# kdavila/lecturemath

Measured on AMD Instinct MI355X. Metric: frames/sec end-to-end binarize+CC+group @1080p, higher is better.
Workload: dtype u8

## Files before the change

lecturemath_amd/csrc/lm_api.hip:

```cpp
#include "lm_common.h"
#include "lm_stream.h"

#include <stdarg.h>
#include <stdlib.h>
#include <stdio.h>
#include <string.h>

#include "../../include/lecturemath_amd.h"

#include "lm_cc_kernels.hip"
#include "lm_fcn_bytes.hip"
#include "lm_match_kernels.hip"
#include "lm_match_batch.hip"
#include "lm_group.hip"
#include "lm_fcn.hip"
#include "lm_fcn2.hip"

static thread_local char g_err[512] = "";

void lm_set_error(const char* fmt, ...)
{
    va_list ap;
    va_start(ap, fmt);
    vsnprintf(g_err, sizeof(g_err), fmt, ap);
// ... 333 lines not shown
        return LM_ERR_ARG;
    }
    const LmGeom g = c->g;
    hipStream_t st = (hipStream_t)stream;
    if ((long long)g.H * ((g.W + 3) / 4) >= (1ll << 24) && d_labels) { lm_set_error("lm_label_batch: frame too large for the label writer (H*W/4 must be < 2^24)"); return LM_ERR_ARG; }
#if !LM_HIP_EMULATED
    {
        LM_HIP(hipFuncSetAttribute((const void*)lm_k_band, hipFuncAttributeMaxDynamicSharedMemorySize, (int)lm_band_smem(c)));
    }
#endif
    if (lm_profile_mark(c, st, true, n_frames)) return LM_ERR_HIP;
    static const int want_parts = [] { const char* e = getenv("LM_LABEL_PARTS"); const int v = e ? atoi(e) : LM_LABEL_PARTS; return (v >= 1 && v <= 8) ? v : LM_LABEL_PARTS; }();
    int parts = want_parts;
    while (parts > 1 && n_frames / parts < LM_LABEL_PART_MIN) parts--;
    if (parts > 1 && !c->aux_stream) {
        LM_HIP(hipStreamCreateWithFlags((hipStream_t*)&c->aux_stream, hipStreamNonBlocking));
        LM_HIP(hipEventCreateWithFlags((hipEvent_t*)&c->ev_fork, hipEventDisableTiming));
        LM_HIP(hipEventCreateWithFlags((hipEvent_t*)&c->ev_join, hipEventDisableTiming));
    }
    if (parts <= 1) {
        const int rc = lm_label_launch(c, src, 0, n_frames, d_labels, st);
        if (rc) return rc;
    } else {
        hipStream_t aux = (hipStream_t)c->aux_stream;
        LM_HIP(hipEventRecord((hipEvent_t)c->ev_fork, st));
        LM_HIP(hipStreamWaitEvent(aux, (hipEvent_t)c->ev_fork, 0));
        int rc = LM_OK;
        for (int k = 0, f0 = 0; k < parts && rc == LM_OK; k++) {
            const int n = n_frames / parts + (k < n_frames % parts ? 1 : 0);
            rc = lm_label_launch(c, src, f0, n, d_labels, (k & 1) ? aux : st);
            f0 += n;
        }
        const hipError_t e1 = hipEventRecord((hipEvent_t)c->ev_join, aux);
        const hipError_t e2 = (e1 == hipSuccess) ? hipStreamWaitEvent(st, (hipEvent_t)c->ev_join, 0) : e1;
        if (e2 != hipSuccess) {
            (void)hipStreamSynchronize(aux);
            if (rc == LM_OK) { lm_set_error("lm_label_batch: joining the second queue failed: %s", hipGetErrorString(e2)); rc = LM_ERR_HIP; }
        }
        if (rc) return rc;
    }
    if (lm_profile_mark(c, st, false, n_frames)) return LM_ERR_HIP;
    c->last_batch = n_frames;
    c->last_fused = src.logits ? 1 : 0;
    c->stats_fresh = 1;
    return LM_OK;
}

extern "C" int lm_label_batch(LmCtx* c, const uint8_t* d_binary, int n_frames, int32_t* d_labels, void* stream)
{
    LmLabelSrc src = {d_binary, nullptr, 0.0f, 0u, nullptr};
    return lm_label_batch_src(c, src, n_frames, d_labels, stream);
}

extern "C" int lm_label_batch_logits(LmCtx* c, const float* d_logits, int n_frames, int thr, int invert, uint8_t* d_binary, int32_t* d_labels, void* stream)
{
    if (!c || !d_logits || n_frames <= 0 || n_frames > c->max_batch) {
        lm_set_error("lm_label_batch_logits: bad arguments (n_frames=%d, max_batch=%d)", n_frames, c ? c->max_batch : -1);
        return LM_ERR_ARG;
    }
    const LmGeom g = c->g;
    float edge = 0.0f;
    int cmp = 0;
    const bool shape_ok = (g.W & 3) == 0 && ((((uintptr_t)d_logits) & 15) == 0) && (!d_binary || ((((uintptr_t)d_binary) & 3) == 0));
    {
        const int rc = lm_threshold_form(shape_ok && !getenv("LM_LABEL_UNFUSED"), thr, (hipStream_t)stream, &edge, &cmp);
        if (rc) return rc;
    }
    if (cmp) {
        LmLabelSrc src = {nullptr, d_logits, edge, invert ? 0xffu : 0u, d_binary};
        return lm_label_batch_src(c, src, n_frames, d_labels, stream);
    }
    if (!d_binary) { lm_set_error("lm_label_batch_logits: this frame shape / threshold needs the two-pass path, which needs d_binary"); return LM_ERR_ARG; }
    const int rc = lm_threshold(d_logits, d_binary, (int64_t)n_frames * g.W * g.H, thr, invert, stream);
    if (rc) return rc;
    return lm_label_batch(c, d_binary, n_frames, d_labels, stream);
}

extern "C" int lm_label_was_fused(LmCtx* c) { return c ? c->last_fused : 0; }

extern "C" int lm_label_counts(LmCtx* c, int32_t* h_counts, void* stream)
{
    if (!c || !h_counts || c->last_batch <= 0) { lm_set_error("lm_label_counts: no labelled batch"); return LM_ERR_STATE; }
    LM_HIP(hipMemcpyAsync(h_counts, c->n_labels, (size_t)c->last_batch * sizeof(int32_t), hipMemcpyDeviceToHost,
                          (hipStream_t)stream));
    LM_HIP(hipStreamSynchronize((hipStream_t)stream));
    if (g_band_stamps && getenv("LM_DEBUG_BAND_STAMPS")) {
        const size_t n = (size_t)c->nbands * c->last_batch * 8;
        unsigned long long* h = (unsigned long long*)malloc(n * sizeof(unsigned long long));
        if (h && hipMemcpy(h, g_band_stamps, n * sizeof(unsigned long long), hipMemcpyDeviceToHost) == hipSuccess) {
            FILE* f = fopen(getenv("LM_DEBUG_BAND_STAMPS"), "wb");
            if (f) { fwrite(h, sizeof(unsigned long long), n, f); fclose(f); }
        }
        free(h);
    }
    return LM_OK;
}

extern "C" int lm_cc_stats_batch(LmCtx* c, void* stream)
{
    if (!c || c->last_batch <= 0) { lm_set_error("lm_cc_stats_batch: no labelled batch"); return LM_ERR_STATE; }
    const LmGeom g = c->g;
    hipStream_t st = (hipStream_t)stream;
    const int B = c->last_batch;
    if (!c->stats_fresh)
        hipLaunchKernelGGL(lm_k_stats_init, dim3(32, B), dim3(256), 0, st, c->st_min_y, c->st_max_y, c->st_min_x, c->st_max_x,
                           c->st_count, c->n_labels, g.W, g.H, g.cap);
    c->stats_fresh = 0;
    hipLaunchKernelGGL(lm_k_stats, dim3((g.WW + LM_ST_WORDS - 1) / LM_ST_WORDS, (g.H + LM_ST_ROWS - 1) / LM_ST_ROWS, B), dim3(256), 0,
                       st, c->bits, c->starts, c->prefix, c->rowoff, c->final_label, c->st_min_y, c->st_max_y, c->st_min_x,
                       c->st_max_x, c->st_count, g.WW, g.H, g.cap);
    LM_HIP(hipGetLastError());
    return LM_OK;
}

extern "C" int lm_cc_stats_read(LmCtx* c, int frame, int n, int32_t* h_mins_y, int32_t* h_maxs_y, int32_t* h_mins_x,
                                int32_t* h_maxs_x, int32_t* h_counts, void* stream)
{
    if (!c || frame < 0 || frame >= c->last_batch || n < 0 || n > c->g.cap) {
        lm_set_error("lm_cc_stats_read: bad arguments");
        return LM_ERR_ARG;
    }
    hipStream_t st = (hipStream_t)stream;
    const size_t off = (size_t)frame * c->g.cap, nb = (size_t)n * sizeof(int32_t);
    if (n > 0) {
        if (h_mins_y) LM_HIP(hipMemcpyAsync(h_mins_y, c->st_min_y + off, nb, hipMemcpyDeviceToHost, st));
        if (h_maxs_y) LM_HIP(hipMemcpyAsync(h_maxs_y, c->st_max_y + off, nb, hipMemcpyDeviceToHost, st));
        if (h_mins_x) LM_HIP(hipMemcpyAsync(h_mins_x, c->st_min_x + off, nb, hipMemcpyDeviceToHost, st));
        if (h_maxs_x) LM_HIP(hipMemcpyAsync(h_maxs_x, c->st_max_x + off, nb, hipMemcpyDeviceToHost, st));
// ... 48 lines not shown
                                int* out_maxs_y, int* out_mins_x, int* out_maxs_x, int* out_counts, float* output_age)
{
    if (count_labels <= 0 || width <= 0 || height <= 0) return 0;
    LmCtx* c = lm_host_ctx(width, height);
    const size_t px = (size_t)width * height;
    if (!c || lm_stage(c, px)) return 0;
    const int n = count_labels;
    int32_t* d_out = nullptr;
    if (hipMalloc((void**)&d_out, (size_t)n * 9 * sizeof(int32_t)) != hipSuccess) { lm_set_error("CC_AgeBoundaries: hipMalloc failed"); return 0; }
    int32_t *mny = d_out, *mxy = d_out + n, *mnx = d_out + 2 * (size_t)n, *mxx = d_out + 3 * (size_t)n, *cnt = d_out + 4 * (size_t)n,
            *ageb = d_out + 5 * (size_t)n, *last_px = d_out + 7 * (size_t)n, *last_neg = d_out + 8 * (size_t)n;
    float* agef = (float*)(d_out + 6 * (size_t)n);
    bool ok = hipMemcpy(c->stage_i32, labels, px * sizeof(int32_t), hipMemcpyHostToDevice) == hipSuccess;
    if (ok && ages) ok = hipMemcpy(c->stage_f32, ages, px * sizeof(float), hipMemcpyHostToDevice) == hipSuccess;
    if (ok) {
        const float* d_ages = ages ? c->stage_f32 : (const float*)nullptr;
        hipLaunchKernelGGL(lm_k_ab_init, dim3(lm_blocks(n, 256)), dim3(256), 0, (hipStream_t)0, mny, mxy, mnx, mxx, cnt, ageb, last_px, last_neg,
                           width, height, n);
        hipLaunchKernelGGL(lm_k_ab_scan, dim3(lm_blocks((long long)px, 256)), dim3(256), 0, (hipStream_t)0, c->stage_i32, d_ages, width, height, n,
                           mny, mxy, mnx, mxx, cnt, last_px, last_neg);
        hipLaunchKernelGGL(lm_k_ab_age, dim3(lm_blocks((long long)px, 256)), dim3(256), 0, (hipStream_t)0, c->stage_i32, d_ages, width, height, n,
                           last_neg, ageb);
        hipLaunchKernelGGL(lm_k_ab_finish, dim3(lm_blocks(n, 256)), dim3(256), 0, (hipStream_t)0, ageb, last_px, last_neg, d_ages, agef, n);
        const size_t nb = (size_t)n * sizeof(int32_t);
        ok = hipMemcpy(out_mins_y, mny, nb, hipMemcpyDeviceToHost) == hipSuccess &&
             hipMemcpy(out_maxs_y, mxy, nb, hipMemcpyDeviceToHost) == hipSuccess &&
             hipMemcpy(out_mins_x, mnx, nb, hipMemcpyDeviceToHost) == hipSuccess &&
             hipMemcpy(out_maxs_x, mxx, nb, hipMemcpyDeviceToHost) == hipSuccess &&
             hipMemcpy(out_counts, cnt, nb, hipMemcpyDeviceToHost) == hipSuccess &&
             hipMemcpy(output_age, agef, nb, hipMemcpyDeviceToHost) == hipSuccess;
    }
    if (!ok) lm_set_error("CC_AgeBoundaries: device copy/launch failed");
    (void)hipFree(d_out);
    return 0;
}

extern "C" void lm_stream_destroy(LmStream* s)
{
    if (!s) return;
    void* ptrs[] = {s->cc, s->assign, s->frame_cc_off, s->crop, s->chash, s->active_cc, s->active_box, s->active_last, s->active, s->counters, s->best,
                    s->batch_cc_base, s->batch_word_base};
    for (void* p : ptrs)
        if (p) (void)hipFree(p);
    if (s->mb) {
        LmMatchBatch* m = s->mb;
        void* mp[] = {m->nt_cnt, m->nt_src, m->tlast, m->tcur[0], m->tcur[1], m->ftile_all, m->nt_foff, m->nt_list, m->cls, m->troot, m->rootpos, m->ftile, m->s_prefix, m->tcount[0], m->tcount[1], m->toff[0], m->toff[1], m->pairs[0], m->pairs[1], m->pair_u[0],
                      m->pair_u[1], m->sidx, m->s_list, m->s_box, m->newpos, m->n_src, m->ttab, m->tkey, m->twin, m->big[0], m->big[1], m->n_big};
        for (void* p : mp)
            if (p) (void)hipFree(p);
        delete m;
    }
    for (int i = 0; i < s->n_run_events; i++) (void)hipEventDestroy(s->run_events[i]);
    free(s->run_events);
    if (s->rd_scratch) (void)hipFree(s->rd_scratch);
    if (s->garena) (void)hipFree(s->garena);
    if (s->gpin) (void)hipHostFree(s->gpin);
    delete s;
}

extern "C" int lm_stream_set_min_pixels(LmStream* s, int min_pixels)
{
    if (!s || min_pixels < 0) { lm_set_error("lm_stream_set_min_pixels: bad arguments"); return LM_ERR_ARG; }
    s->min_pixels = min_pixels;
    return LM_OK;
}

extern "C" int lm_stream_reset(LmStream* s, void* stream)
{
    if (!s) { lm_set_error("lm_stream_reset: null stream"); return LM_ERR_ARG; }
    LM_HIP(hipMemsetAsync(s->counters, 0, sizeof(LmCounters), (hipStream_t)stream));
    LM_HIP(hipMemsetAsync(s->best, 0xff, (size_t)s->ctx->g.cap * sizeof(unsigned long long), (hipStream_t)stream));
    LM_HIP(hipMemsetAsync(s->frame_cc_off, 0, sizeof(long long), (hipStream_t)stream));
    LM_HIP(hipMemsetAsync(s->chash, 0, (size_t)s->cap_cc * sizeof(uint32_t), (hipStream_t)stream));
    if (s->mb) LM_HIP(hipMemsetAsync(s->mb->ttab, 0xff, (size_t)LM_MB_TTAB * sizeof(unsigned long long), (hipStream_t)stream));
    s->frames_pushed = 0;
    s->frames_matched = 0;
    s->tempo_B = 0;
    return LM_OK;
}

extern "C" LmStream* lm_stream_create(LmCtx* ctx, int max_frames, int64_t max_ccs, int64_t max_crop_words, int max_uniques,
                                      double min_recall, double min_precision, int max_gap, int min_pixels)
{
    if (!ctx || max_frames <= 0 || max_ccs <= 0 || max_crop_words <= 0 || max_uniques <= 0) {
        lm_set_error("lm_stream_create: bad arguments");
        return nullptr;
    }
    LmStream* s = new LmStream();
    memset(s, 0, sizeof(*s));
    s->ctx = ctx;
    s->cap_frames = max_frames;
    s->cap_cc = max_ccs;
    s->cap_words = (unsigned long long)max_crop_words;
    s->cap_uniq = max_uniques;
    s->min_recall = min_recall;
    s->min_precision = min_precision;
    s->max_gap = max_gap;
    s->min_pixels = min_pixels;
    int rc = LM_OK;
    rc |= lm_alloc(&s->cc, (size_t)max_ccs);
    rc |= lm_alloc(&s->assign, (size_t)max_ccs);
    rc |= lm_alloc(&s->frame_cc_off, (size_t)max_frames + 1);
    rc |= lm_alloc(&s->crop, (size_t)max_crop_words);
    rc |= lm_alloc(&s->chash, (size_t)max_ccs);
    rc |= lm_alloc(&s->active_cc, (size_t)max_uniques);
    rc |= lm_alloc(&s->active_box, (size_t)max_uniques);
    rc |= lm_alloc(&s->active_last, (size_t)max_uniques);
    rc |= lm_alloc(&s->active, (size_t)max_uniques);
    rc |= lm_alloc(&s->best, (size_t)ctx->g.cap);
    rc |= lm_alloc(&s->counters, (size_t)1);
    rc |= lm_alloc(&s->batch_cc_base, (size_t)ctx->max_batch);
    rc |= lm_alloc(&s->batch_word_base, (size_t)ctx->max_batch);
    {
        LmMatchBatch* m = new LmMatchBatch();
        memset(m, 0, sizeof(*m));
        s->mb = m;
        m->cap_tiles = (int)(max_ccs / LM_MB_TILE) + max_frames + 2;
        long long cp = 16 * (long long)max_ccs;
        if (cp < (1 << 16)) cp = 1 << 16;
        if (cp > (1 << 23)) cp = 1 << 23;
        m->cap_pairs = (uint32_t)cp;
        rc |= lm_alloc(&m->ftile, (size_t)max_frames + 2);
        rc |= lm_alloc(&m->s_prefix, (size_t)max_frames + 2);
        rc |= lm_alloc(&m->ftile_all, (size_t)max_frames + 2);
        rc |= lm_alloc(&m->nt_foff, (size_t)max_frames + 2);
        rc |= lm_alloc(&m->nt_list, (size_t)max_ccs);
        rc |= lm_alloc(&m->cls, (size_t)max_ccs);
        rc |= lm_alloc(&m->troot, (size_t)max_ccs);
        rc |= lm_alloc(&m->rootpos, (size_t)max_ccs);
        rc |= lm_alloc(&m->nt_cnt, (size_t)LM_MB_MAX_FRAMES);
        rc |= lm_alloc(&m->nt_src, (size_t)max_ccs);
        rc |= lm_alloc(&m->tlast, (size_t)max_ccs);
        for (int k = 0; k < 2; k++) {
            rc |= lm_alloc(&m->tcount[k], (size_t)m->cap_tiles + 1);
            rc |= lm_alloc(&m->toff[k], (size_t)m->cap_tiles + 1);
            rc |= lm_alloc(&m->tcur[k], ((size_t)m->cap_tiles + 1) * LM_MB_JY);
            rc |= lm_alloc(&m->pairs[k], (size_t)m->cap_pairs);
            rc |= lm_alloc(&m->pair_u[k], (size_t)m->cap_pairs);
        }
        rc |= lm_alloc(&m->sidx, (size_t)max_ccs);
        rc |= lm_alloc(&m->s_list, (size_t)max_ccs);
        rc |= lm_alloc(&m->s_box, (size_t)max_ccs);
        rc |= lm_alloc(&m->newpos, (size_t)max_ccs);
        rc |= lm_alloc(&m->n_src, (size_t)1);
        rc |= lm_alloc(&m->ttab, (size_t)LM_MB_TTAB);
        rc |= lm_alloc(&m->tkey, (size_t)max_ccs);
        rc |= lm_alloc(&m->twin, (size_t)max_ccs);
        m->cap_big = 1u << 16;
        rc |= lm_alloc(&m->big[0], (size_t)m->cap_big);
        rc |= lm_alloc(&m->big[1], (size_t)m->cap_big);
        rc |= lm_alloc(&m->n_big, (size_t)2);
#if !LM_HIP_EMULATED
        if (rc == LM_OK &&
            hipFuncSetAttribute((const void*)lm_k_mb_resolve, hipFuncAttributeMaxDynamicSharedMemorySize, (int)LM_MB_RESOLVE_SMEM) != hipSuccess)
            rc = LM_ERR_HIP;
#endif
        const char* e = getenv("LM_MATCH_PER_FRAME");
        s->match_per_frame = (e && atoi(e) == 1) ? 1 : 0;
    }
    if (rc == LM_OK && hipMemset(s->mb->twin, 0, (size_t)max_ccs) != hipSuccess) rc = LM_ERR_HIP;
    if (rc == LM_OK) rc = lm_stream_reset(s, nullptr);
    if (rc == LM_OK && hipStreamSynchronize(nullptr) != hipSuccess) rc = LM_ERR_HIP;
    if (rc != LM_OK) {
        lm_stream_destroy(s);
        return nullptr;
    }
    return s;
}

static void lm_launch_match(LmStream* s, int f, hipStream_t st)
{
    hipLaunchKernelGGL(lm_k_match, LM_HIP_EMULATED ? dim3(2, 2) : dim3(16, 64), dim3(256), 0, st, s->cc, s->crop, s->frame_cc_off, f,
                       s->active_box, s->active_last, s->active_cc, s->counters, s->best, s->min_recall, s->min_precision, s->max_gap);
    hipLaunchKernelGGL(lm_k_update, dim3(1), dim3(1024), 0, st, s->cc, s->frame_cc_off, f, s->active, s->active_cc, s->active_box,
                       s->active_last, s->counters, s->assign, s->best, s->max_gap, s->cap_uniq, (f & 15) == 15 ? 1 : 0);
}

static void lm_flush_tempo(LmStream* s, hipStream_t st)
{
    if (s->tempo_B <= 0) return;
    const LmMatchBatch mb = *s->mb;
    hipLaunchKernelGGL(lm_k_mb_tempo, dim3(LM_HIP_EMULATED ? 2 : 1024), dim3(256), 0, st, s->cc, s->frame_cc_off, s->tempo_f0, s->tempo_B, s->active_box,
                       s->active_cc, s->active_last, s->counters, mb, s->max_gap, s->active, s->assign);
    s->tempo_B = 0;
}

static void lm_launch_match_frames(LmStream* s, int f0, int n, hipStream_t st, hipEvent_t ev_pre = nullptr, bool defer_tempo = false)
{
    if (!s->match_per_frame) lm_flush_tempo(s, st);
    if (s->match_per_frame) {
        for (int i = 0; i < n; i++) lm_launch_match(s, f0 + i, st);
        return;
    }
    const LmMatchBatch mb = *s->mb;
    const dim3 gj(LM_HIP_EMULATED ? 2 : 128, LM_HIP_EMULATED ? 2 : LM_MB_JY), gt(LM_HIP_EMULATED ? 2 : 1024), ge(LM_HIP_EMULATED ? 2 : 2048), gb(LM_HIP_EMULATED ? 2 : 1024);
    for (int done = 0; done < n;) {
        const int B = (n - done < LM_MB_MAX_FRAMES) ? n - done : LM_MB_MAX_FRAMES;
        const int f = f0 + done;
        s->last_match_frames = B;
        const int twins = (s->min_recall <= 1.0 && s->min_precision <= 1.0) ? 1 : 0;
        if (twins) {
            const dim3 gc(LM_HIP_EMULATED ? 2 : 256);
            hipLaunchKernelGGL(lm_k_mb_twin_insert, gc, dim3(256), 0, st, s->cc, s->chash, s->frame_cc_off, f, B, s->counters, mb);
            hipLaunchKernelGGL(lm_k_mb_twin_probe, gc, dim3(256), 0, st, s->cc, s->frame_cc_off, f, B, s->counters, mb, s->max_gap);
            hipLaunchKernelGGL(lm_k_mb_twin_cmp, ge, dim3(256), 0, st, s->cc, s->crop, s->frame_cc_off, f, B, s->counters, mb);
            hipLaunchKernelGGL(lm_k_mb_twin_final, gc, dim3(256), 0, st, s->cc, s->frame_cc_off, f, B, s->counters, mb);
        }
        hipLaunchKernelGGL(lm_k_mb_nt, dim3(B + 1), dim3(1024), 0, st, s->frame_cc_off, f, B, s->active, s->active_cc, s->active_box, s->active_last,
                           s->counters, mb, s->max_gap, twins);
        hipLaunchKernelGGL((lm_k_mb_join<0, 0>), gj, dim3(256), 0, st, s->cc, s->frame_cc_off, f, B, s->active_box, s->active_cc, s->counters, mb);
        hipLaunchKernelGGL((lm_k_mb_join<0, 1>), gj, dim3(256), 0, st, s->cc, s->frame_cc_off, f, B, s->active_box, s->active_cc, s->counters, mb);
        hipLaunchKernelGGL((lm_k_mb_eval<0>), ge, dim3(256), 0, st, s->cc, s->crop, s->frame_cc_off, f, B, s->active_last, s->counters, mb,
                           s->min_recall, s->min_precision, s->max_gap);
        hipLaunchKernelGGL((lm_k_mb_eval_big<0>), gb, dim3(256), 0, st, s->cc, s->crop, s->active_last, s->counters, mb, s->min_recall, s->min_precision,
                           s->max_gap);
        hipLaunchKernelGGL(lm_k_mb_sources, dim3(1), dim3(1024), 0, st, s->cc, s->frame_cc_off, f, B, s->counters, mb);
        hipLaunchKernelGGL((lm_k_mb_join<1, 0>), gj, dim3(256), 0, st, s->cc, s->frame_cc_off, f, B, s->active_box, s->active_cc, s->counters, mb);
        hipLaunchKernelGGL((lm_k_mb_join<1, 1>), gj, dim3(256), 0, st, s->cc, s->frame_cc_off, f, B, s->active_box, s->active_cc, s->counters, mb);
        hipLaunchKernelGGL((lm_k_mb_eval<1>), ge, dim3(256), 0, st, s->cc, s->crop, s->frame_cc_off, f, B, s->active_last, s->counters, mb,
                           s->min_recall, s->min_precision, s->max_gap);
        hipLaunchKernelGGL((lm_k_mb_eval_big<1>), gb, dim3(256), 0, st, s->cc, s->crop, s->active_last, s->counters, mb, s->min_recall, s->min_precision,
                           s->max_gap);
        if (ev_pre && done + B >= n) (void)hipEventRecord(ev_pre, st);
        hipLaunchKernelGGL(lm_k_mb_resolve, dim3(1), dim3(LM_MB_RT), LM_MB_RESOLVE_SMEM, st, s->cc, s->frame_cc_off, f, B, s->active, s->active_cc,
                           s->active_box, s->active_last, s->counters, s->assign, mb, s->max_gap, s->cap_uniq);
        if (defer_tempo && done + B >= n) { s->tempo_f0 = f; s->tempo_B = B; }
        else
            hipLaunchKernelGGL(lm_k_mb_tempo, gt, dim3(256), 0, st, s->cc, s->frame_cc_off, f, B, s->active_box, s->active_cc, s->active_last,
                               s->counters, mb, s->max_gap, s->active, s->assign);
        done += B;
    }
}

static int lm_stream_emit_batch(LmStream* s, int B, void* stream)
{
    LmCtx* c = s->ctx;
    const LmGeom g = c->g;
    hipStream_t st = (hipStream_t)stream;
    int rc = lm_cc_stats_batch(c, stream);
    if (rc) return rc;
    hipLaunchKernelGGL(lm_k_select, dim3(B), dim3(1024), 0, st, c->st_min_y, c->st_max_y, c->st_min_x, c->st_max_x,
                       c->st_count, c->n_labels, c->kept_label, c->kept_cropoff, c->frame_kept, c->frame_cropwords, g.cap,
                       s->min_pixels);
    hipLaunchKernelGGL(lm_k_batch_offsets, dim3(1), dim3(1024), 0, st, c->frame_kept, c->frame_cropwords, B, s->counters,
                       s->frame_cc_off, s->batch_cc_base, s->batch_word_base, s->cap_cc, s->cap_words, s->cap_frames);
    hipLaunchKernelGGL(lm_k_emit, dim3(LM_HIP_EMULATED ? 2 : LM_EMIT_GRID, B), dim3(256), 0, st, c->bits, c->starts, c->prefix, c->rowoff, c->final_label,
                       c->st_min_y, c->st_max_y, c->st_min_x, c->st_max_x, c->st_count, c->kept_label, c->kept_cropoff,
                       c->frame_kept, c->frame_cropwords, s->batch_cc_base, s->batch_word_base, s->cc, s->crop, s->chash, s->frames_pushed, g.WW,
                       g.H, g.cap);
    LM_HIP(hipGetLastError());
    return LM_OK;
}

extern "C" int lm_stream_push_labelled(LmStream* s, int n_frames, void* stream)
{
    if (!s || n_frames <= 0 || n_frames != s->ctx->last_batch) {
        lm_set_error("lm_stream_push_labelled: %d frames, the context's last labelled batch has %d", n_frames, s ? s->ctx->last_batch : 0);
        return LM_ERR_ARG;
    }
    if (s->frames_pushed + n_frames > s->cap_frames) {
// ... 31 lines not shown
            lm_launch_match_frames(s, s->frames_pushed, B, st);
            s->frames_matched += B;
        }
        LM_HIP(hipGetLastError());
        s->frames_pushed += B;
        done += B;
    }
    return LM_OK;
}

extern "C" int lm_stream_push(LmStream* s, const uint8_t* d_binary, int n_frames, int32_t* d_labels, void* stream)
{
    return lm_stream_push_impl(s, d_binary, n_frames, d_labels, 1, stream);
}

extern "C" int lm_stream_push_records(LmStream* s, const uint8_t* d_binary, int n_frames, int32_t* d_labels, void* stream)
{
    return lm_stream_push_impl(s, d_binary, n_frames, d_labels, 0, stream);
}

static int lm_run_events(LmStream* s, int want)
{
    if (want <= s->n_run_events) return LM_OK;
    want += 192;
    hipEvent_t* ev = (hipEvent_t*)realloc(s->run_events, (size_t)want * sizeof(hipEvent_t));
    if (!ev) { lm_set_error("lm_stream_run_logits: out of memory"); return LM_ERR_HIP; }
    s->run_events = ev;
    for (; s->n_run_events < want; s->n_run_events++) LM_HIP(hipEventCreateWithFlags(&s->run_events[s->n_run_events], hipEventDisableTiming));
    return LM_OK;
}

extern "C" int lm_stream_run_logits(LmStream* s, const float* d_logits, int n_frames, int batch, uint8_t* d_binary, int32_t* d_labels, int thr,
                                    int do_match, int schedule, void* stream_wide, void* stream_match)
{
    if (!s || !d_logits || n_frames < 0 || batch <= 0 || batch > s->ctx->max_batch || schedule < 0 || schedule > 1) {
        lm_set_error("lm_stream_run_logits: bad arguments (batch %d, context batch %d, schedule %d)", batch, s ? s->ctx->max_batch : 0, schedule);
        return LM_ERR_ARG;
    }
    if (do_match && s->frames_matched != s->frames_pushed) {
        lm_set_error("lm_stream_run_logits: %d frames pushed without matching; call lm_stream_match first", s->frames_pushed - s->frames_matched);
        return LM_ERR_STATE;
    }
    hipStream_t sw = (hipStream_t)stream_wide, sm = (hipStream_t)stream_match;
    const bool two = do_match && sm != sw;
    const bool gated = two && schedule == 1 && batch <= LM_MB_MAX_FRAMES && !s->match_per_frame;
    const size_t px = (size_t)s->ctx->g.W * s->ctx->g.H;
    const int nb = (n_frames + batch - 1) / batch;
    if (two) { const int rc = lm_run_events(s, 3 * nb); if (rc) return rc; }
    hipEvent_t* ev = s->run_events;
    int prev_n = 0;
    for (int k = 0, f0 = 0; f0 < n_frames; f0 += batch, k++) {
        const int n = (n_frames - f0 < batch) ? n_frames - f0 : batch;
        if (gated && k >= 2) LM_HIP(hipStreamWaitEvent(sw, ev[3 * (k - 2) + 2], 0));
        int rc = lm_label_batch_logits(s->ctx, d_logits + (size_t)f0 * px, n, thr, 1, d_binary, d_labels, stream_wide);
        if (rc) return rc;
        if (gated) LM_HIP(hipEventRecord(ev[3 * k], sw));
        rc = lm_stream_push_labelled(s, n, stream_wide);
        if (rc) return rc;
        if (!do_match) continue;
        if (!two) {
            rc = lm_stream_match(s, n, stream_wide);
            if (rc) return rc;
        } else if (!gated) {
            LM_HIP(hipEventRecord(ev[3 * k + 1], sw));
            LM_HIP(hipStreamWaitEvent(sm, ev[3 * k + 1], 0));
            rc = lm_stream_match(s, n, stream_match);
            if (rc) return rc;
        } else {
            LM_HIP(hipEventRecord(ev[3 * k + 1], sw));
            if (k >= 1) {
                LM_HIP(hipStreamWaitEvent(sm, ev[3 * k], 0));
                lm_launch_match_frames(s, s->frames_matched, prev_n, sm, ev[3 * (k - 1) + 2], true);
                s->frames_matched += prev_n;
            }
        }
        prev_n = n;
    }
    if (gated && nb > 0) {
        LM_HIP(hipStreamWaitEvent(sm, ev[3 * (nb - 1) + 1], 0));
        lm_launch_match_frames(s, s->frames_matched, prev_n, sm, ev[3 * (nb - 1) + 2]);
        s->frames_matched += prev_n;
    }
    lm_flush_tempo(s, sm);
    LM_HIP(hipGetLastError());
    return LM_OK;
}

extern "C" int lm_stream_match(LmStream* s, int n_frames, void* stream)
{
    if (!s || n_frames < 0 || s->frames_matched + n_frames > s->frames_pushed) {
        lm_set_error("lm_stream_match: %d frames requested, %d pushed, %d matched", n_frames, s ? s->frames_pushed : 0, s ? s->frames_matched : 0);
        return LM_ERR_ARG;
    }
    lm_launch_match_frames(s, s->frames_matched, n_frames, (hipStream_t)stream);
    s->frames_matched += n_frames;
    LM_HIP(hipGetLastError());
    return LM_OK;
}

extern "C" int lm_stream_match_stats(LmStream* s, int64_t* out5, void* stream)
{
    if (!s || !out5 || !s->mb) { lm_set_error("lm_stream_match_stats: bad arguments"); return LM_ERR_ARG; }
    hipStream_t st = (hipStream_t)stream;
    const LmMatchBatch* m = s->mb;
    const int B = s->last_match_frames;
    int32_t nsrc = 0, nt = 0;
    uint32_t ta = 0, tb = 0;
    if (B > 0) {
        LM_HIP(hipMemcpyAsync(&nsrc, m->n_src, 4, hipMemcpyDeviceToHost, st));
        LM_HIP(hipMemcpyAsync(&nt, m->ftile + B, 4, hipMemcpyDeviceToHost, st));
        LM_HIP(hipStreamSynchronize(st));
        if (nt > 0) {
            LM_HIP(hipMemcpyAsync(&ta, m->toff[0] + nt, 4, hipMemcpyDeviceToHost, st));
            LM_HIP(hipMemcpyAsync(&tb, m->toff[1] + nt, 4, hipMemcpyDeviceToHost, st));
            LM_HIP(hipStreamSynchronize(st));
        }
    }
    out5[0] = nsrc; out5[1] = nt; out5[2] = ta; out5[3] = tb; out5[4] = B;
    return LM_OK;
}

__global__ void __launch_bounds__(1024) lm_k_compact_active(int32_t* __restrict__ active, int32_t* __restrict__ active_cc,
// ... 396 lines not shown
```

lecturemath_amd/csrc/lm_match_batch.hip:

```cpp
#include "lm_stream.h"

#define LM_MB_TILE 64
#define LM_MB_JY 8
#define LM_MB_TTAB (1 << 18)
#ifndef LM_MB_CHUNK
#define LM_MB_CHUNK 1024
#endif
#define LM_MB_MAX_FRAMES 64
#define LM_MB_BIGPAIR 2048
#ifndef LM_MB_CH
#define LM_MB_CH 2048
#endif
#define LM_MB_LA 16384
#define LM_MB_LS 16384
#ifndef LM_MB_PFA
#define LM_MB_PFA 2
#endif
#ifndef LM_MB_PFB
#define LM_MB_PFB 1
#endif
#define LM_MB_RESOLVE_SMEM ((size_t)LM_MB_CH * 8 + (size_t)LM_MB_LA * 4 + (size_t)LM_MB_LS * 4)

struct LmMatchBatch {
    int32_t* ftile;
// ... 60 lines not shown
        unsigned kept = 0;
        for (int base = 0; base < nA; base += 1024 * LM_UPD_ITEMS) {
            int32_t u[LM_UPD_ITEMS], uc[LM_UPD_ITEMS], ul[LM_UPD_ITEMS];
            unsigned long long ub[LM_UPD_ITEMS];
            unsigned keep[LM_UPD_ITEMS], mine = 0;
#pragma unroll
            for (int k = 0; k < LM_UPD_ITEMS; k++) {
                int i = base + (int)threadIdx.x * LM_UPD_ITEMS + k;
                keep[k] = 0;
                if (i < nA) {
                    u[k] = active[i]; uc[k] = active_cc[i]; ub[k] = active_box[i]; ul[k] = active_last[i];
                    keep[k] = lm_mb_alive(f0, ul[k], max_gap) ? 1u : 0u;
                }
                mine += keep[k];
            }
            unsigned tot;
            unsigned ex = lm_block_excl_scan<1024>(mine, &tot);
            unsigned o = kept + ex;
#pragma unroll
            for (int k = 0; k < LM_UPD_ITEMS; k++)
                if (keep[k]) { active[o] = u[k]; active_cc[o] = uc[k]; active_box[o] = ub[k]; active_last[o] = ul[k]; o++; }
            kept += tot;
        }
        nA = (int)kept;
    }
    if (threadIdx.x == 0) {
        *mb.n_src = 0;
        cnt->n_active = nA;
    }
}

#define LM_MB_NT_R 4

__global__ void __launch_bounds__(1024) lm_k_mb_nt(const long long* __restrict__ frame_cc_off, int f0, int B, int32_t* __restrict__ active,
                                                   int32_t* __restrict__ active_cc, unsigned long long* __restrict__ active_box,
                                                   int32_t* __restrict__ active_last, LmCounters* __restrict__ cnt, LmMatchBatch mb, int max_gap,
                                                   int twins)
{
    __shared__ unsigned s_tab[LM_MB_NT_R * 16];
    __shared__ unsigned s_tot;
    __shared__ int s_head[6];
    if (cnt->error) return;
    if ((int)blockIdx.x == B) {
        if (threadIdx.x < 2) mb.n_big[threadIdx.x] = 0;
        lm_mb_prologue(frame_cc_off, f0, B, active, active_cc, active_box, active_last, cnt, mb, max_gap);
        return;
    }
    const int b = (int)blockIdx.x;
    const int lane = lm_lane(), wid = (int)(threadIdx.x >> 6);
    if (wid == 0) {
        unsigned n_nt = 0, n_all = 0;
        if (lane < B) {
            n_all = (unsigned)(frame_cc_off[f0 + lane + 1] - frame_cc_off[f0 + lane]);
            n_nt = twins ? (unsigned)mb.nt_cnt[lane] : n_all;
        }
        const unsigned t_nt = (n_nt + LM_MB_TILE - 1) / LM_MB_TILE, t_all = (n_all + LM_MB_TILE - 1) / LM_MB_TILE;
        const unsigned i_nt = lm_wave_incl_scan(n_nt), i_tnt = lm_wave_incl_scan(t_nt), i_tall = lm_wave_incl_scan(t_all);
        if (lane == b) {
            s_head[0] = (int)(i_nt - n_nt); s_head[1] = (int)(i_tnt - t_nt); s_head[2] = (int)i_tnt;
            mb.nt_foff[b] = (int32_t)(i_nt - n_nt);
            mb.ftile[b] = (int32_t)(i_tnt - t_nt);
            mb.ftile_all[b] = (int32_t)(i_tall - t_all);
            if (b == B - 1) {
                mb.nt_foff[B] = (int32_t)i_nt;
                mb.ftile[B] = (int32_t)i_tnt;
                mb.ftile_all[B] = (int32_t)i_tall;
                if ((int)i_tnt > mb.cap_tiles || (int)i_tall > mb.cap_tiles) cnt->error = LM_ERR_CAPACITY;
            }
        }
    }
    __syncthreads();
    const int t0 = s_head[1], t1 = s_head[2] + (b == B - 1 ? 1 : 0);
    for (int t = t0 + (int)threadIdx.x; t < t1 && t <= mb.cap_tiles; t += 1024) { mb.tcount[0][t] = 0; mb.tcount[1][t] = 0; }
    const long long C0 = frame_cc_off[f0 + b], C1 = frame_cc_off[f0 + b + 1];
    unsigned carry = (unsigned)s_head[0];
    for (long long base = C0; base < C1; base += 1024 * LM_MB_NT_R) {
        unsigned fm = 0;
#pragma unroll
        for (int k = 0; k < LM_MB_NT_R; k++) {
            const long long i = base + (long long)k * 1024 + threadIdx.x;
            const int flag = (i < C1) ? (mb.twin[i] == 0) : 0;
            fm |= (unsigned)flag << k;
            const unsigned long long bal = __ballot(flag);
            if (lane == 0) s_tab[k * 16 + wid] = (unsigned)__popcll(bal);
        }
        __syncthreads();
        if (wid == 0) {
            const unsigned v = s_tab[lane];
            const unsigned incl = lm_wave_incl_scan(v);
            s_tab[lane] = incl - v;
            if (lane == 63) s_tot = incl;
        }
        __syncthreads();
#pragma unroll
        for (int k = 0; k < LM_MB_NT_R; k++) {
            const int flag = (int)((fm >> k) & 1u);
            const unsigned long long bal = __ballot(flag);
            const long long i = base + (long long)k * 1024 + threadIdx.x;
            if (flag) {
                const unsigned o = carry + s_tab[k * 16 + wid] + (unsigned)__popcll(bal & lm_lowmask_excl(lane));
                mb.nt_list[o] = (int32_t)i; mb.cls[i] = (int32_t)o; mb.tlast[o] = -1; mb.sidx[i] = -2;
            }
        }
        carry += s_tot;
        __syncthreads();
    }
}
// ... 175 lines not shown
        const bool deferred = big && slot < mb.cap_big;
        if (deferred && sub == 0) mb.big[SRC][slot] = p;
        if (live && possible && !deferred) {
            for (int y = is.y0 + sub; y <= is.y1; y += 8) {
                const unsigned long long ra = rec.crop_off + (unsigned long long)((y - rec.min_y) * is.anw + (is.wc0 - is.awx0));
                const unsigned long long ru = urec.crop_off + (unsigned long long)((y - urec.min_y) * is.unw + (is.wc0 - is.uwx0));
                for (int j = 0; j < is.nwc; j++) m += __popc(crop[ra + j] & crop[ru + j]);
            }
        }
#pragma unroll
        for (int d = 4; d >= 1; d >>= 1) m += __shfl_xor(m, d, 8);
        if (live && possible && !deferred && sub == 0 && lm_accept(m, rec.size, urec.size, min_recall, min_precision)) {
            mb.pairs[SRC][p].x = pr.x | 0x80000000u;
            if (SRC == 0 && lm_mb_alive(rec.frame, active_last[pr.y], max_gap)) mb.sidx[ci] = -1;
        }
    }
}

template <int SRC>
__global__ void __launch_bounds__(256) lm_k_mb_eval_big(const LmCcRec* __restrict__ cc, const uint32_t* __restrict__ crop,
                                                        const int32_t* __restrict__ active_last, LmCounters* __restrict__ cnt, LmMatchBatch mb,
                                                        double min_recall, double min_precision, int max_gap)
{
    __shared__ int s_sum;
    if (cnt->error) return;
    const unsigned n = mb.n_big[SRC] < mb.cap_big ? mb.n_big[SRC] : mb.cap_big;
    for (unsigned b = blockIdx.x; b < n; b += gridDim.x) {
        const unsigned p = mb.big[SRC][b];
        const uint2 pr = mb.pairs[SRC][p];
        const long long ci = (long long)mb.nt_list[pr.x];
        const LmCcRec rec = cc[ci], urec = cc[mb.pair_u[SRC][p]];
        const LmIsect is = lm_isect(rec, urec);
        if (threadIdx.x == 0) s_sum = 0;
        __syncthreads();
        int m = lm_overlap_words(rec, urec, is, crop, (int)threadIdx.x, 256);
        m = lm_wave_sum(m);
        if (lm_lane() == 0 && m) atomicAdd(&s_sum, m);
        __syncthreads();
        if (threadIdx.x == 0 && lm_accept(s_sum, rec.size, urec.size, min_recall, min_precision)) {
            mb.pairs[SRC][p].x = pr.x | 0x80000000u;
            if (SRC == 0 && lm_mb_alive(rec.frame, active_last[pr.y], max_gap)) mb.sidx[ci] = -1;
        }
        __syncthreads();
    }
}

__global__ void __launch_bounds__(256) lm_k_mb_twin_insert(const LmCcRec* __restrict__ cc, const uint32_t* __restrict__ chash,
                                                           const long long* __restrict__ frame_cc_off, int f0, int B,
                                                           LmCounters* __restrict__ cnt, LmMatchBatch mb)
{
    if (cnt->error) return;
    const long long C0 = frame_cc_off[f0], C1 = frame_cc_off[f0 + B];
    const long long n = C1 - C0;
    if (blockIdx.x == 0 && threadIdx.x < LM_MB_MAX_FRAMES) mb.nt_cnt[threadIdx.x] = 0;
    if (n * 2 > LM_MB_TTAB) return;
    for (long long i = (long long)blockIdx.x * blockDim.x + threadIdx.x; i < n; i += (long long)gridDim.x * blockDim.x) {
        const LmCcRec r = cc[C0 + i];
        const unsigned h = chash[C0 + i];
        const unsigned long long box = lm_pack_box(r);
        unsigned key = lm_mix32(h ^ lm_mix32((unsigned)box) ^ lm_mix32((unsigned)(box >> 32) + 0x85ebca6bu) ^ lm_mix32((unsigned)r.size + 0xc2b2ae35u));
        if (key == 0xffffffffu) key = 0;
        mb.tkey[C0 + i] = key;
        const unsigned long long val = ((unsigned long long)key << 32) | (unsigned long long)(unsigned)i;
        for (unsigned probe = 0; probe < LM_MB_TTAB; probe++) {
            const unsigned slot = (key + probe) & (LM_MB_TTAB - 1);
            const unsigned long long old = atomicCAS(&mb.ttab[slot], ~0ull, val);
            if (old == ~0ull) break;
            if ((unsigned)(old >> 32) == key) { atomicMin(&mb.ttab[slot], val); break; }
        }
    }
}

__global__ void __launch_bounds__(256) lm_k_mb_twin_probe(const LmCcRec* __restrict__ cc, const long long* __restrict__ frame_cc_off, int f0, int B,
                                                          LmCounters* __restrict__ cnt, LmMatchBatch mb, int max_gap)
{
    if (cnt->error) return;
    const long long C0 = frame_cc_off[f0], C1 = frame_cc_off[f0 + B];
    const long long n = C1 - C0;
    const bool enabled = n * 2 <= LM_MB_TTAB;
    for (long long i = (long long)blockIdx.x * blockDim.x + threadIdx.x; i < n; i += (long long)gridDim.x * blockDim.x) {
        long long root = -1;
        if (enabled) {
            const unsigned key = mb.tkey[C0 + i];
            for (unsigned probe = 0; probe < LM_MB_TTAB; probe++) {
                const unsigned slot = (key + probe) & (LM_MB_TTAB - 1);
                const unsigned long long e = mb.ttab[slot];
                if (e == ~0ull) break;
                if ((unsigned)(e >> 32) == key) {
                    root = (long long)(unsigned)e;
                    mb.tkey[C0 + i] = slot;
                    break;
                }
            }
            if (root >= 0 && root < i) {
                const LmCcRec r = cc[C0 + i], q = cc[C0 + root];
                if (!(r.size == q.size && r.min_x == q.min_x && r.max_x == q.max_x && r.min_y == q.min_y && r.max_y == q.max_y &&
                      q.frame < r.frame && r.frame - q.frame <= max_gap))
                    root = -1;
            } else {
                root = -1;
            }
        }
        mb.twin[C0 + i] = root >= 0 ? 1 : 0;
        mb.troot[C0 + i] = root >= 0 ? (int32_t)(C0 + root) : -1;
    }
}

// ... 65 lines not shown
        if (tid == 0) s_off[nwin] = (klo + nwin < n) ? cc[C0 + klo + nwin].crop_off : W1;
        __syncthreads();
        const unsigned long long wend = s_off[nwin] < wb1 ? s_off[nwin] : wb1;
        if (s_any) {
            for (unsigned long long w0 = cur + (unsigned long long)(tid & ~63) * LM_TW_UNR; w0 < wend; w0 += STEP) {
                int jj[LM_TW_UNR];
                unsigned mine[LM_TW_UNR], theirs[LM_TW_UNR];
#pragma unroll
                for (int u = 0; u < LM_TW_UNR; u++) {
                    const unsigned long long w = w0 + (unsigned long long)(u * 64 + lane);
                    jj[u] = -1; mine[u] = 0; theirs[u] = 0;
                    if (w < wend) {
                        int lo = 0, hi = nwin;
                        while (hi - lo > 1) {
                            const int mid = (lo + hi) >> 1;
                            if (s_off[mid] <= w) lo = mid; else hi = mid;
                        }
                        if (s_root[lo] >= 0) {
                            jj[u] = lo;
                            mine[u] = crop[w];
                            theirs[u] = crop[s_roff[lo] + (w - s_off[lo])];
                        }
                    }
                }
#pragma unroll
                for (int u = 0; u < LM_TW_UNR; u++)
                    if (jj[u] >= 0 && mine[u] != theirs[u]) mb.twin[C0 + klo + jj[u]] = 0;
            }
        }
        cur = wend;
        klo += nwin;
    }
}

__global__ void __launch_bounds__(256) lm_k_mb_twin_final(const LmCcRec* __restrict__ cc, const long long* __restrict__ frame_cc_off, int f0, int B,
                                                          LmCounters* __restrict__ cnt, LmMatchBatch mb)
{
    if (cnt->error) return;
    const long long C0 = frame_cc_off[f0], C1 = frame_cc_off[f0 + B];
    const int lane = lm_lane();
    if ((C1 - C0) * 2 <= LM_MB_TTAB)
        for (long long i = C0 + (long long)blockIdx.x * blockDim.x + threadIdx.x; i < C1; i += (long long)gridDim.x * blockDim.x)
            mb.ttab[mb.tkey[i] & (LM_MB_TTAB - 1)] = ~0ull;
    for (long long base = C0 + ((long long)blockIdx.x * blockDim.x + (threadIdx.x & ~63u)); base < C1; base += (long long)gridDim.x * blockDim.x) {
        const long long i = base + lane;
        const bool nt = i < C1 && !mb.twin[i];
        int fb = -1;
        if (nt) { mb.troot[i] = -1; fb = cc[i].frame - f0; }
        unsigned long long todo = __ballot(nt);
        while (todo) {
            const int leader = __ffsll((long long)todo) - 1;
            const int fl = __shfl(fb, leader);
            const unsigned long long same = __ballot(nt && fb == fl);
            if (lane == leader) atomicAdd(&mb.nt_cnt[fl], (int)__popcll(same));
            todo &= ~same;
        }
    }
}

__global__ void __launch_bounds__(256) lm_k_crop_hash(const LmCcRec* __restrict__ cc, const uint32_t* __restrict__ crop, long long c0, long long n,
                                                      unsigned long long W1, uint32_t* __restrict__ chash)
{
    if (n <= 0) return;
    const unsigned long long W0 = cc[c0].crop_off;
    const int lane = lm_lane();
    const unsigned long long wave = ((unsigned long long)blockIdx.x * blockDim.x + threadIdx.x) >> 6, nwaves = ((unsigned long long)gridDim.x * blockDim.x) >> 6;
    for (unsigned long long w0 = W0 + wave * 64ull; w0 < W1; w0 += nwaves * 64ull) {
        const long long k0 = lm_cc_of_word_search(cc, c0, n, w0);
        const unsigned long long w = w0 + (unsigned long long)lane;
        const bool live = w < W1;
        long long k = k0;
        unsigned contrib = 0;
        if (live) {
            k = lm_cc_of_word(cc, c0, n, w, k0);
            contrib = lm_mix32(crop[w] + 0x9e3779b9u * (unsigned)(w - cc[c0 + k].crop_off));
        }
        const bool same = live && k == k0;
        const unsigned wsum = lm_wave_sum(same ? contrib : 0u);
        if (lane == 0 && live) atomicAdd(&chash[c0 + k0], wsum);
        if (live && !same) atomicAdd(&chash[c0 + k], contrib);
    }
}

#define LM_MB_SRC_R 8

__global__ void __launch_bounds__(1024) lm_k_mb_sources(const LmCcRec* __restrict__ cc, const long long* __restrict__ frame_cc_off,
                                                        int f0, int B, LmCounters* __restrict__ cnt, LmMatchBatch mb)
{
    __shared__ unsigned s_tab[LM_MB_SRC_R * 16];
    __shared__ unsigned s_tot;
    if (cnt->error) return;
    const int nNT = mb.nt_foff[B];
    const int lane = lm_lane(), wid = (int)(threadIdx.x >> 6);
    unsigned carry = 0;
    for (int base = 0; base < nNT; base += 1024 * LM_MB_SRC_R) {
        int ci[LM_MB_SRC_R], v[LM_MB_SRC_R];
#pragma unroll
        for (int k = 0; k < LM_MB_SRC_R; k++) {
            const int e = base + k * 1024 + (int)threadIdx.x;
            ci[k] = (e < nNT) ? mb.nt_list[e] : -1;
        }
#pragma unroll
        for (int k = 0; k < LM_MB_SRC_R; k++) v[k] = (ci[k] >= 0) ? mb.sidx[ci[k]] : 0;
        unsigned fm = 0;
#pragma unroll
        for (int k = 0; k < LM_MB_SRC_R; k++) {
            const int flag = v[k] == -2;
// ... 362 lines not shown
```

lecturemath_amd/csrc/lm_stream.h:

```cpp
#pragma once
#include "lm_common.h"

struct __attribute__((aligned(32))) LmCcRec {
    int32_t cc_id;
    int32_t size;
    int16_t min_x, max_x, min_y, max_y;
    unsigned long long crop_off;
    int32_t frame;
    int32_t pad;
};

struct LmCounters {
    long long n_cc;
    unsigned long long n_words;
    unsigned long long tempo_count;
    int n_frames;
    int n_matched;
    int n_uniq;
    int n_active;
    int error;
    int pad;
};

struct LmStream {
    LmCtx* ctx;
    long long cap_cc;
    unsigned long long cap_words;
    int cap_frames, cap_uniq;
    double min_recall, min_precision;
    int max_gap, min_pixels;
    LmCcRec* cc;
    int32_t* assign;
    long long* frame_cc_off;
    uint32_t* crop;
    uint32_t* chash;
    int32_t* active;
    int32_t* active_cc;
    unsigned long long* active_box;
    int32_t* active_last;
    unsigned long long* best;
    LmCounters* counters;
    long long* batch_cc_base;
    unsigned long long* batch_word_base;
    void* rd_scratch;
    size_t rd_scratch_bytes;
    void* garena;
    size_t garena_bytes;
    int garena_busy;
    void* gpin;
    size_t gpin_bytes;
    int gpin_busy;
    struct LmMatchBatch* mb;
    int last_match_frames;
    int match_per_frame;
    hipEvent_t* run_events;
    int n_run_events;
    int tempo_f0, tempo_B;
    int frames_pushed;
    int frames_matched;
};
```

Before: 75320.

## Launch twin-detection kernels early on the wide stream and skip binary output

Twin-detection kernels (insert/probe/cmp/final) for a batch are now launched on the wide stream right after a push, ahead of the match stage. The match stage skips them when a recorded mark shows they already ran. The per-frame nt_cnt buffer is now indexed by absolute frame, sized max_frames, so early results survive until match consumes them. The end-to-end path also stops writing the binarized frames in the fused labelling path, which removes a store. This adds bookkeeping and cross-stream event ordering that must stay consistent.

```diff
diff --git a/lecturemath_amd/csrc/lm_api.hip b/lecturemath_amd/csrc/lm_api.hip
--- a/lecturemath_amd/csrc/lm_api.hip
+++ b/lecturemath_amd/csrc/lm_api.hip
@@ -409,7 +409,8 @@
     return lm_label_batch_src(c, src, n_frames, d_labels, stream);
 }
 
-extern "C" int lm_label_batch_logits(LmCtx* c, const float* d_logits, int n_frames, int thr, int invert, uint8_t* d_binary, int32_t* d_labels, void* stream)
+static int lm_label_logits_impl(LmCtx* c, const float* d_logits, int n_frames, int thr, int invert, uint8_t* d_binary, bool keep_frames,
+                                int32_t* d_labels, void* stream)
 {
     if (!c || !d_logits || n_frames <= 0 || n_frames > c->max_batch) {
         lm_set_error("lm_label_batch_logits: bad arguments (n_frames=%d, max_batch=%d)", n_frames, c ? c->max_batch : -1);
@@ -418,19 +419,25 @@
     const LmGeom g = c->g;
     float edge = 0.0f;
     int cmp = 0;
-    const bool shape_ok = (g.W & 3) == 0 && ((((uintptr_t)d_logits) & 15) == 0) && (!d_binary || ((((uintptr_t)d_binary) & 3) == 0));
+    uint8_t* const d_out = keep_frames ? d_binary : nullptr;
+    const bool shape_ok = (g.W & 3) == 0 && ((((uintptr_t)d_logits) & 15) == 0) && (!d_out || ((((uintptr_t)d_out) & 3) == 0));
     {
         const int rc = lm_threshold_form(shape_ok && !getenv("LM_LABEL_UNFUSED"), thr, (hipStream_t)stream, &edge, &cmp);
         if (rc) return rc;
     }
     if (cmp) {
-        LmLabelSrc src = {nullptr, d_logits, edge, invert ? 0xffu : 0u, d_binary};
+        LmLabelSrc src = {nullptr, d_logits, edge, invert ? 0xffu : 0u, d_out};
         return lm_label_batch_src(c, src, n_frames, d_labels, stream);
     }
     if (!d_binary) { lm_set_error("lm_label_batch_logits: this frame shape / threshold needs the two-pass path, which needs d_binary"); return LM_ERR_ARG; }
     const int rc = lm_threshold(d_logits, d_binary, (int64_t)n_frames * g.W * g.H, thr, invert, stream);
     if (rc) return rc;
     return lm_label_batch(c, d_binary, n_frames, d_labels, stream);
+}
+
+extern "C" int lm_label_batch_logits(LmCtx* c, const float* d_logits, int n_frames, int thr, int invert, uint8_t* d_binary, int32_t* d_labels, void* stream)
+{
+    return lm_label_logits_impl(c, d_logits, n_frames, thr, invert, d_binary, true, d_labels, stream);
 }
 
 extern "C" int lm_label_was_fused(LmCtx* c) { return c ? c->last_fused : 0; }
@@ -585,6 +592,7 @@
     }
     for (int i = 0; i < s->n_run_events; i++) (void)hipEventDestroy(s->run_events[i]);
     free(s->run_events);
+    if (s->twin_ev) (void)hipEventDestroy(s->twin_ev);
     if (s->rd_scratch) (void)hipFree(s->rd_scratch);
     if (s->garena) (void)hipFree(s->garena);
     if (s->gpin) (void)hipHostFree(s->gpin);
@@ -609,6 +617,8 @@
     s->frames_pushed = 0;
     s->frames_matched = 0;
     s->tempo_B = 0;
+    s->n_twin_marks = 0;
+    s->twin_done_to = 0;
     return LM_OK;
 }
 
@@ -661,7 +671,7 @@
         rc |= lm_alloc(&m->cls, (size_t)max_ccs);
         rc |= lm_alloc(&m->troot, (size_t)max_ccs);
         rc |= lm_alloc(&m->rootpos, (size_t)max_ccs);
-        rc |= lm_alloc(&m->nt_cnt, (size_t)LM_MB_MAX_FRAMES);
+        rc |= lm_alloc(&m->nt_cnt, (size_t)max_frames);
         rc |= lm_alloc(&m->nt_src, (size_t)max_ccs);
         rc |= lm_alloc(&m->tlast, (size_t)max_ccs);
         for (int k = 0; k < 2; k++) {
@@ -691,6 +701,7 @@
         const char* e = getenv("LM_MATCH_PER_FRAME");
         s->match_per_frame = (e && atoi(e) == 1) ? 1 : 0;
     }
+    if (rc == LM_OK && hipEventCreateWithFlags(&s->twin_ev, hipEventDisableTiming) != hipSuccess) rc = LM_ERR_HIP;
     if (rc == LM_OK && hipMemset(s->mb->twin, 0, (size_t)max_ccs) != hipSuccess) rc = LM_ERR_HIP;
     if (rc == LM_OK) rc = lm_stream_reset(s, nullptr);
     if (rc == LM_OK && hipStreamSynchronize(nullptr) != hipSuccess) rc = LM_ERR_HIP;
@@ -718,6 +729,55 @@
     s->tempo_B = 0;
 }
 
+static bool lm_stream_twins(const LmStream* s) { return s->min_recall <= 1.0 && s->min_precision <= 1.0; }
+
+static void lm_launch_twins(LmStream* s, int f, int B, hipStream_t st)
+{
+    if (s->twin_last_ev && s->twin_last_stream != st) (void)hipStreamWaitEvent(st, s->twin_last_ev, 0);
+    const LmMatchBatch mb = *s->mb;
+    const dim3 gc(LM_HIP_EMULATED ? 2 : 256), ge(LM_HIP_EMULATED ? 2 : 2048);
+    hipLaunchKernelGGL(lm_k_mb_twin_insert, gc, dim3(256), 0, st, s->cc, s->chash, s->frame_cc_off, f, B, s->counters, mb);
+    hipLaunchKernelGGL(lm_k_mb_twin_probe, gc, dim3(256), 0, st, s->cc, s->frame_cc_off, f, B, s->counters, mb, s->max_gap);
+    hipLaunchKernelGGL(lm_k_mb_twin_cmp, ge, dim3(256), 0, st, s->cc, s->crop, s->frame_cc_off, f, B, s->counters, mb);
+    hipLaunchKernelGGL(lm_k_mb_twin_final, gc, dim3(256), 0, st, s->cc, s->frame_cc_off, f, B, s->counters, mb);
+    s->twin_last_stream = st;
+    s->twin_last_ev = nullptr;
+}
+
+static void lm_twins_follow(LmStream* s, hipEvent_t ev)
+{
+    if (!ev) { ev = s->twin_ev; (void)hipEventRecord(ev, s->twin_last_stream); }
+    s->twin_last_ev = ev;
+}
+
+static bool lm_launch_twins_ahead(LmStream* s, int f0, int n, hipStream_t st)
+{
+    if (s->match_per_frame || !lm_stream_twins(s)) return false;
+    const int chunks = (n + LM_MB_MAX_FRAMES - 1) / LM_MB_MAX_FRAMES;
+    if (f0 != s->twin_done_to || s->n_twin_marks + chunks > LM_TWIN_MARKS) return false;
+    for (int done = 0; done < n;) {
+        const int B = (n - done < LM_MB_MAX_FRAMES) ? n - done : LM_MB_MAX_FRAMES;
+        lm_launch_twins(s, f0 + done, B, st);
+        s->twin_mark[s->n_twin_marks][0] = f0 + done;
+        s->twin_mark[s->n_twin_marks][1] = B;
+        s->n_twin_marks++;
+        done += B;
+    }
+    s->twin_done_to = f0 + n;
+    return true;
+}
+
+static bool lm_twins_were_ahead(LmStream* s, int f, int B)
+{
+    if (s->n_twin_marks > 0 && s->twin_mark[0][0] == f && s->twin_mark[0][1] == B) {
+        s->n_twin_marks--;
+        memmove(&s->twin_mark[0][0], &s->twin_mark[1][0], (size_t)s->n_twin_marks * sizeof(s->twin_mark[0]));
+        return true;
+    }
+    s->n_twin_marks = 0;
+    return false;
+}
+
 static void lm_launch_match_frames(LmStream* s, int f0, int n, hipStream_t st, hipEvent_t ev_pre = nullptr, bool defer_tempo = false)
 {
     if (!s->match_per_frame) lm_flush_tempo(s, st);
@@ -731,14 +791,9 @@
         const int B = (n - done < LM_MB_MAX_FRAMES) ? n - done : LM_MB_MAX_FRAMES;
         const int f = f0 + done;
         s->last_match_frames = B;
-        const int twins = (s->min_recall <= 1.0 && s->min_precision <= 1.0) ? 1 : 0;
-        if (twins) {
-            const dim3 gc(LM_HIP_EMULATED ? 2 : 256);
-            hipLaunchKernelGGL(lm_k_mb_twin_insert, gc, dim3(256), 0, st, s->cc, s->chash, s->frame_cc_off, f, B, s->counters, mb);
-            hipLaunchKernelGGL(lm_k_mb_twin_probe, gc, dim3(256), 0, st, s->cc, s->frame_cc_off, f, B, s->counters, mb, s->max_gap);
-            hipLaunchKernelGGL(lm_k_mb_twin_cmp, ge, dim3(256), 0, st, s->cc, s->crop, s->frame_cc_off, f, B, s->counters, mb);
-            hipLaunchKernelGGL(lm_k_mb_twin_final, gc, dim3(256), 0, st, s->cc, s->frame_cc_off, f, B, s->counters, mb);
-        }
+        const int twins = lm_stream_twins(s) ? 1 : 0;
+        if (twins && !lm_twins_were_ahead(s, f, B)) { lm_launch_twins(s, f, B, st); lm_twins_follow(s, nullptr); }
+        if (s->twin_done_to < f + B) s->twin_done_to = f + B;
         hipLaunchKernelGGL(lm_k_mb_nt, dim3(B + 1), dim3(1024), 0, st, s->frame_cc_off, f, B, s->active, s->active_cc, s->active_box, s->active_last,
                            s->counters, mb, s->max_gap, twins);
         hipLaunchKernelGGL((lm_k_mb_join<0, 0>), gj, dim3(256), 0, st, s->cc, s->frame_cc_off, f, B, s->active_box, s->active_cc, s->counters, mb);
@@ -876,22 +931,25 @@
     for (int k = 0, f0 = 0; f0 < n_frames; f0 += batch, k++) {
         const int n = (n_frames - f0 < batch) ? n_frames - f0 : batch;
         if (gated && k >= 2) LM_HIP(hipStreamWaitEvent(sw, ev[3 * (k - 2) + 2], 0));
-        int rc = lm_label_batch_logits(s->ctx, d_logits + (size_t)f0 * px, n, thr, 1, d_binary, d_labels, stream_wide);
+        int rc = lm_label_logits_impl(s->ctx, d_logits + (size_t)f0 * px, n, thr, 1, d_binary, false, d_labels, stream_wide);
         if (rc) return rc;
         if (gated) LM_HIP(hipEventRecord(ev[3 * k], sw));
         rc = lm_stream_push_labelled(s, n, stream_wide);
         if (rc) return rc;
         if (!do_match) continue;
+        {
+            const bool ahead = lm_launch_twins_ahead(s, s->frames_pushed - n, n, sw);
+            if (two) LM_HIP(hipEventRecord(ev[3 * k + 1], sw));
+            if (ahead) lm_twins_follow(s, two ? ev[3 * k + 1] : nullptr);
+        }
         if (!two) {
             rc = lm_stream_match(s, n, stream_wide);
             if (rc) return rc;
         } else if (!gated) {
-            LM_HIP(hipEventRecord(ev[3 * k + 1], sw));
             LM_HIP(hipStreamWaitEvent(sm, ev[3 * k + 1], 0));
             rc = lm_stream_match(s, n, stream_match);
             if (rc) return rc;
         } else {
-            LM_HIP(hipEventRecord(ev[3 * k + 1], sw));
             if (k >= 1) {
                 LM_HIP(hipStreamWaitEvent(sm, ev[3 * k], 0));
                 lm_launch_match_frames(s, s->frames_matched, prev_n, sm, ev[3 * (k - 1) + 2], true);
diff --git a/lecturemath_amd/csrc/lm_match_batch.hip b/lecturemath_amd/csrc/lm_match_batch.hip
--- a/lecturemath_amd/csrc/lm_match_batch.hip
+++ b/lecturemath_amd/csrc/lm_match_batch.hip
@@ -136,7 +136,7 @@
         unsigned n_nt = 0, n_all = 0;
         if (lane < B) {
             n_all = (unsigned)(frame_cc_off[f0 + lane + 1] - frame_cc_off[f0 + lane]);
-            n_nt = twins ? (unsigned)mb.nt_cnt[lane] : n_all;
+            n_nt = twins ? (unsigned)mb.nt_cnt[f0 + lane] : n_all;
         }
         const unsigned t_nt = (n_nt + LM_MB_TILE - 1) / LM_MB_TILE, t_all = (n_all + LM_MB_TILE - 1) / LM_MB_TILE;
         const unsigned i_nt = lm_wave_incl_scan(n_nt), i_tnt = lm_wave_incl_scan(t_nt), i_tall = lm_wave_incl_scan(t_all);
@@ -418,7 +418,7 @@
     if (cnt->error) return;
     const long long C0 = frame_cc_off[f0], C1 = frame_cc_off[f0 + B];
     const long long n = C1 - C0;
-    if (blockIdx.x == 0 && threadIdx.x < LM_MB_MAX_FRAMES) mb.nt_cnt[threadIdx.x] = 0;
+    if (blockIdx.x == 0 && (int)threadIdx.x < B) mb.nt_cnt[f0 + threadIdx.x] = 0;
     if (n * 2 > LM_MB_TTAB) return;
     for (long long i = (long long)blockIdx.x * blockDim.x + threadIdx.x; i < n; i += (long long)gridDim.x * blockDim.x) {
         const LmCcRec r = cc[C0 + i];
@@ -590,7 +590,7 @@
             const int leader = __ffsll((long long)todo) - 1;
             const int fl = __shfl(fb, leader);
             const unsigned long long same = __ballot(nt && fb == fl);
-            if (lane == leader) atomicAdd(&mb.nt_cnt[fl], (int)__popcll(same));
+            if (lane == leader) atomicAdd(&mb.nt_cnt[f0 + fl], (int)__popcll(same));
             todo &= ~same;
         }
     }
diff --git a/lecturemath_amd/csrc/lm_stream.h b/lecturemath_amd/csrc/lm_stream.h
--- a/lecturemath_amd/csrc/lm_stream.h
+++ b/lecturemath_amd/csrc/lm_stream.h
@@ -1,5 +1,7 @@
 #pragma once
 #include "lm_common.h"
+
+#define LM_TWIN_MARKS 8
 
 struct __attribute__((aligned(32))) LmCcRec {
     int32_t cc_id;
@@ -56,6 +58,12 @@
     hipEvent_t* run_events;
     int n_run_events;
     int tempo_f0, tempo_B;
+    int twin_mark[LM_TWIN_MARKS][2];
+    int n_twin_marks;
+    int twin_done_to;
+    hipEvent_t twin_ev;
+    hipEvent_t twin_last_ev;
+    hipStream_t twin_last_stream;
     int frames_pushed;
     int frames_matched;
 };
```

New measurement: 76390 (median of 6 runs). 1.4% higher.
